# bigpon/QPNet

Hardware: AMD Instinct MI355X
Metric: train steps/sec (batch-1 chunk-steps of RF+20000 samples, aggregate over GPUs) (higher is better)
Workload: dtype f32; 1 GPU; config[1]: paper-size SI-QPNet (C=64,S=256,4F+4A) training step, forward+CE+backward+Adam on one chunk of 20900 samples (RF 946 + batch_length 19954), batch 1 per GPU; global_batch=1, parallelism=dp1 (utterance-sharded chunks, one flat-gradient all-reduce per step), backend=none, world_size=1, aux_1x1=frame rate (hoisted: K = 128 + one 4-deep step)

## Files before the change

qpnet_amd/csrc/train_common.h:

```cpp
#pragma once
#include "qpn_common.h"

typedef float f32x4 __attribute__((ext_vector_type(4)));

#define TR_MAXL QPN_MAX_LAYERS

__host__ __device__ static inline int tr_lda(int K) { return ((K + 29) / 32) * 32 + 2; }
__host__ __device__ static inline int tr_ldt(int N) { return ((N + 15) / 32) * 32 + 16; }

struct TrLayer {
    int adaptive, dilation;
    int s_in, s_out;
    int tap_off;
    int w1_f4, wr_f4;
    int w1t_f4, wrt_f4;
    int bias1, biasr;
};

struct TrainParams {
    int C, S, Q, A, Ap, L, U;
    int B, T, F, Td, BL, N1, N0, maxd;
    int Kt, Ktp;
    int LC;
    const float* flat;
// ... 21 lines not shown
    int qtotal;
    int qP[TR_MAXL + 1];
    int qT[TR_MAXL];
    int ws_f4, p1_f4, p2_f4;
    int wst_f4, p1t_f4, p2t_f4;
    int bias_s, bias_p1, bias_p2;
    int64_t causal_w, causal_b, up_w, up_b;
    TrLayer layers[TR_MAXL];
};

struct TrainSlabs {
    int g_w1[TR_MAXL], g_b1[TR_MAXL], g_wr[TR_MAXL], g_br[TR_MAXL], g_ws[TR_MAXL], g_bs;
    int g_p1, g_bp1, g_p2, g_bp2;
    int g_early0, g_early1;
    int g_cw, g_cb;
};

struct TrainBwd {
    const float* dlogits; float* gflat;
    float* DXA[2]; float* DXB[2];
    float* DZ;
    float* DS0; float* DY0;
    float* DGS;
    float* DHUP;
    float* DPA;
    float* GW;
    float* EB;
    float* slab;
    const int* gdst; const int* gdst_list;
    const int* gzero; int n_gzero;
    int nch, gstage;
    int64_t n_params;
    const struct TrainSlabs* sl;
    float gscale;
    int append_scale;
    const int* status;
    hipStream_t side; hipEvent_t ev_fork, ev_join, ev_mid;
    hipEvent_t ev_early; int* early_recorded;
};


struct AuxGeom { int auxS[TR_MAXL], auxT[TR_MAXL], bias1[TR_MAXL], s_out[TR_MAXL]; };
struct AuxArgs {
    const float* flat; const float* h; float* PA; float* bp; const float* DPA; const float* EB; const float* GW; float* gflat;
    float gscale; int C, A, L, B, F, U, N1, nfr, ffirst; int64_t up_w, up_b;
    AuxGeom g;
};
static inline AuxArgs tr_aux_args(const TrainParams& p, const TrainBwd* bw, const AuxGeom& ag) {
    AuxArgs a; a.flat = p.flat; a.h = p.h; a.PA = p.PA; a.bp = p.bp; a.DPA = bw ? bw->DPA : nullptr; a.EB = bw ? bw->EB : nullptr; a.GW = bw ? bw->GW : nullptr;
    a.gflat = bw ? bw->gflat : nullptr; a.gscale = bw ? bw->gscale : 1.f;
    a.C = p.C; a.A = p.A; a.L = p.L; a.B = p.B; a.F = p.F; a.U = p.U; a.N1 = p.N1; a.nfr = p.nfr; a.ffirst = p.ffirst; a.up_w = p.up_w; a.up_b = p.up_b; a.g = ag;
    return a;
}
struct TrainKnobs {
    bool serial;
    bool stack_q_fwd, stack_q_bwd;
    int stack_wgs, stack_wgs_bwd;
    bool persist_fwd, persist_bwd;
    bool wgrad_generic;
    int wgrad_chunks, wgrad_chunks_side;
    bool post_fuse;
    bool up_side, reduce_early, wr_side;
    bool post_pair, zero_in_post, post_wide;
    bool xcd_swizzle;
    bool ce_separate;
    bool event_fence;
    bool aux_hoist;
    bool test_stack_gives_up;
};
void qpn_train_knobs_parse(TrainKnobs& k);

#define TR_QHEAD_STRIDE 1056
#define TR_QHDR_WORDS 17920
struct StackQ {
    unsigned* flags;
    unsigned* head;
    unsigned* stats;
    unsigned* abort;
    const int4* tab;
    unsigned epoch;
    unsigned epoch_pub;
    unsigned spin_limit;
    int total, nq;
};

__host__ __device__ __forceinline__ int tr_pa_off(const TrainParams& p, int l, int b, int n0) {
    const int q = p.F * p.U - p.N1 + n0;
    return ((l * p.B + b) * (p.nfr + 1) + (q / p.U - p.ffirst)) * 2 * p.C;
}

__device__ __forceinline__ void tr_queue_entry_fwd(const TrainParams& p, int pos, int4& a, int4& b) {
    const bool valid = pos < p.qtotal;
    const int ps = valid ? pos : 0;
    int l = 0;
    for (int k = 1; k < p.L; ++k) l += ps >= p.qP[k] ? 1 : 0;
    const int r = ps - p.qP[l], T = p.qT[l];
    const int bi = r / T, t = r - bi * T;
    const TrLayer ly = p.layers[l];
    const int n0 = ly.s_out + 16 * t;
    int first = 0, n = 0;
    if (valid && l > 0) {
        const int reach = ly.s_out - ly.s_in, s_prev = p.layers[l - 1].s_out;
        int lo = n0 - reach; if (lo < s_prev) lo = s_prev;
        int hi = n0 + 15; if (hi > p.N1 - 1) hi = p.N1 - 1;
        const int t_lo = (lo - s_prev) >> 4, t_hi = (hi - s_prev) >> 4;
        first = p.qP[l - 1] + bi * p.qT[l - 1] + t_lo; n = t_hi - t_lo + 1;
    }
    a = make_int4(n0, l | (bi << 8) | (l == p.L - 1 ? 1 << 24 : 0) | (valid ? 1 << 25 : 0), first, n);
    b = make_int4((l * p.B + bi) * p.N1, ly.tap_off + bi * p.N1, p.hoist ? tr_pa_off(p, l, bi, n0) : bi * p.N1, 0);
}

__device__ __forceinline__ void tr_queue_entry_bwd(const TrainParams& p, int pos, int4& a, int4& b) {
    const bool valid = pos < p.qtotal;
    const int ps = valid ? pos : 0;
    int k = 0, base = 0;
    for (int j = 0; j + 1 < p.L; ++j) { const int n = p.B * p.qT[p.L - 1 - j]; if (ps >= base + n) { base += n; k = j + 1; } else break; }
    const int l = p.L - 1 - k;
    const int r = ps - base, T = p.qT[l];
    const int bi = r / T, t = r - bi * T;
// ... 233 lines not shown
```

qpnet_amd/csrc/train_fwd.hip:

```cpp
#include "train_common.h"
#include "train_post.h"

__device__ __forceinline__ float sigmoidf_(float z) { return __builtin_amdgcn_rcpf(1.0f + __expf(-z)); }
__device__ __forceinline__ float tanhf_(float z) { return 2.0f * __builtin_amdgcn_rcpf(1.0f + __expf(-2.0f * z)) - 1.0f; }

#define AUXP_FPB 8
__device__ __forceinline__ void aux_proj_block(const TrainParams& p, const AuxGeom& ag, int fxb, int l, int b, float* sm) {
    const int fx0 = fxb * AUXP_FPB, tid = threadIdx.x, n = tid & 127, fh = tid >> 7, C = p.C, A = p.A, CA = C * A;
    float* Va = sm; float* hs = sm + 2 * CA;
    {
        const float* s0 = p.flat + ag.auxS[l]; const float* s1 = p.flat + ag.auxT[l];
        for (int base = 0; base < 2 * CA; base += 256 * 16) {
            float v[16];
#pragma unroll
            for (int k = 0; k < 16; ++k) { const int i = base + 256 * k + tid, ic = i < 2 * CA ? i : 0; v[k] = ic < CA ? s0[ic] : s1[ic - CA]; }
#pragma unroll
            for (int k = 0; k < 16; ++k) { const int i = base + 256 * k + tid; if (i < 2 * CA) Va[i] = v[k]; }
        }
    }
    for (int i = tid; i < A * AUXP_FPB; i += 256) {
        const int a = i / AUXP_FPB, f = i - a * AUXP_FPB, fx = fx0 + f;
        hs[i] = fx < p.nfr ? p.h[((size_t)b * A + a) * p.F + p.ffirst + fx] : 0.f;
    }
    __syncthreads();
    float acc[4] = {0.f, 0.f, 0.f, 0.f}, vs = 0.f;
    for (int a = 0; a < A; ++a) {
        const float v = Va[n * A + a];
        const float4 h4 = *(const float4*)(hs + a * AUXP_FPB + 4 * fh);
        acc[0] += v * h4.x; acc[1] += v * h4.y; acc[2] += v * h4.z; acc[3] += v * h4.w;
        vs += v;
    }
    float* out = p.PA + ((size_t)(l * p.B + b) * (p.nfr + 1) + fx0 + 4 * fh) * 2 * C + n;
#pragma unroll
    for (int f = 0; f < 4; ++f) if (fx0 + 4 * fh + f <= p.nfr) out[(size_t)f * 2 * C] = acc[f];
    if (fxb == 0 && b == 0 && fh == 0) p.bp[ag.bias1[l] + n] += p.flat[p.up_b] * vs;
}

__global__ __launch_bounds__(256) void k_train_prep(TrainParams p, AuxGeom ag, int nprep) {
    const int b = blockIdx.y;
    if ((int)blockIdx.x >= nprep) {
        extern __shared__ float sm[];
        const int idx = blockIdx.x - nprep, nfxb = (p.nfr + 1 + AUXP_FPB - 1) / AUXP_FPB;
        aux_proj_block(p, ag, idx % nfxb, idx / nfxb, b, sm);
        return;
    }
    const int C = p.C, Q = p.Q, N1 = p.N1, Ap = p.Ap;
    const int C4 = C / 4, A4 = Ap / 4;
    const int nX = N1 * C4, nH = p.hoist ? 0 : N1 * A4;
    const int total = nX + nH + N1 * p.L;
    if (p.hoist && b == 0)
        for (int n = blockIdx.x * 256 + threadIdx.x; n < N1 + 16; n += nprep * 256) {
            const int q = p.F * p.U - N1 + n, j = q - (q / p.U) * p.U;
            p.WJ[n] = make_float2(p.flat[p.up_w + j], __int_as_float(j));
        }
    if (p.qctl && blockIdx.x == 0 && b == 0 && threadIdx.x < 32) p.qctl[threadIdx.x < 16 ? threadIdx.x : 1024 + (threadIdx.x - 16) * TR_QHEAD_STRIDE] = 0u;
    if (p.qtab && b == 0)
        for (int pos = blockIdx.x * 256 + threadIdx.x; pos <= p.qtotal; pos += nprep * 256) {
            int4 ea, eb; tr_queue_entry_fwd(p, pos, ea, eb);
            p.qtab[2 * pos] = ea; p.qtab[2 * pos + 1] = eb;
            if (p.qtab_b) { tr_queue_entry_bwd(p, pos, ea, eb); p.qtab_b[2 * pos] = ea; p.qtab_b[2 * pos + 1] = eb; }
        }
    for (int it = blockIdx.x * 256 + threadIdx.x; it < total; it += nprep * 256) {
        if (it < nX) {
            const int n = it / C4, c = (it - n * C4) * 4;
            const int64_t xo = (int64_t)p.T - p.N0 + n;
            int64_t s0 = p.x[(size_t)b * p.T + xo] % Q, s1 = p.x[(size_t)b * p.T + xo + 1] % Q;
            if (s0 < 0) s0 += Q;
            if (s1 < 0) s1 += Q;
            const float4 r0 = *(const float4*)(p.ct + (size_t)s0 * C + c);
            const float4 r1 = *(const float4*)(p.ct + ((size_t)Q + s1) * C + c);
            const float4 bb = *(const float4*)(p.flat + p.causal_b + c);
            float4 v;
            v.x = (r0.x + r1.x) + bb.x; v.y = (r0.y + r1.y) + bb.y; v.z = (r0.z + r1.z) + bb.z; v.w = (r0.w + r1.w) + bb.w;
            *(float4*)(p.X + ((size_t)b * N1 + n) * C + c) = v;
            if (c == 0) { p.XC[(size_t)b * (N1 + 1) + n] = (int)s0; if (n == N1 - 1) p.XC[(size_t)b * (N1 + 1) + N1] = (int)s1; }
        } else if (it < nX + nH) {
            const int i2 = it - nX, n = i2 / A4, a0 = (i2 - n * A4) * 4;
            float v[4];
            int64_t f = 0; int j = 0;
            if (p.U > 0) { const int64_t q = (int64_t)p.F * p.U - N1 + n; f = q / p.U; j = (int)(q - f * p.U); }
            else f = (int64_t)p.F - N1 + n;
            const float wj = p.U > 0 ? p.flat[p.up_w + j] : 1.0f, ub = p.U > 0 ? p.flat[p.up_b] : 0.0f;
#pragma unroll
            for (int e = 0; e < 4; ++e) {
                const int a = a0 + e;
                float t = 0.0f;
                if (a < p.A) { t = p.h[((size_t)b * p.A + a) * p.F + f]; if (p.U > 0) t = t * wj + ub; }
                v[e] = t;
            }
            *(float4*)(p.HUP + ((size_t)b * N1 + n) * Ap + a0) = make_float4(v[0], v[1], v[2], v[3]);
        } else {
            const int i3 = it - nX - nH, l = i3 / N1, n = i3 - l * N1;
            const TrLayer ly = p.layers[l];
            int tap;
            if (ly.adaptive) {
                const float dv = p.d[(size_t)b * p.Td + (p.Td - N1 + n)];
                const float dil = -dv * (float)ly.dilation;
                const float s = __fadd_rn(dil, (float)(n - N1));
                tap = N1 + (int)rintf(s);
                if (n >= ly.s_out && (tap < ly.s_in || tap > n)) { atomicOr(p.status, 1); }
            } else tap = n - ly.dilation;
            tap = tap < 0 ? 0 : (tap >= N1 ? N1 - 1 : tap);
            p.TAP[ly.tap_off + (size_t)b * N1 + n] = tap;
        }
    }
}

template <int MT>
__device__ __forceinline__ void layer_fwd_tile(const TrainParams& p, const int l, const int last, const int b, const int n0, float* sm) {
    constexpr int TM = 16 * MT;
    const TrLayer ly = p.layers[l];
    const int C = p.C, Ktp = p.Ktp, Ap = p.Ap;
    const int lda = tr_lda(Ktp), ldg = tr_lda(C);
    float* As = sm; float* Gs = sm + TM * lda;
    const int tid = threadIdx.x, lane = tid & 63, wave = tid >> 6;
    const float* Xin = p.X + ((size_t)(l * p.B + b) * p.N1) * C;
    const float* hup = p.HUP + (size_t)b * p.N1 * Ap;
    const int* taps = p.TAP + ly.tap_off + (size_t)b * p.N1;
    const float* bias1 = p.bp + ly.bias1;
    const float* br = p.bp + ly.biasr;
    const int cpre = 16 * (wave < C / 16 ? wave : 0) + (lane & 15);
    const float bs_pre = bias1[cpre], bt_pre = bias1[C + cpre], bb_pre = br[cpre];
    float4 wrq[4][1];
    if (!last) { const int ntp[1] = {wave < C / 16 ? wave : 0}; wave_b_preload<1, 4>(wrq, p.wp + ly.wr_f4, C / 16, ntp, C, lane); }
    {
        const int K4 = Ktp / 4;
        const int tpr = K4 < 64 ? K4 : 64;
        const int rpp = 256 / tpr;
        const int tr = tid / tpr, tc = tid - tr * tpr;
        constexpr int NR = TM / 4;
        if (tr < rpp) {
            int tp[NR];
#pragma unroll
            for (int k = 0; k < NR; ++k) {
                const int n = n0 + tr + k * rpp;
                tp[k] = taps[n < p.N1 ? n : p.N1 - 1];
            }
            for (int c4 = tc; c4 < K4; c4 += tpr) {
                const int k0 = c4 * 4;
                const int kind = k0 < C ? 0 : k0 < 2 * C ? 1 : k0 < 2 * C + Ap ? 2 : 3;
                const bool from_x = kind <= 1;
                const int col = kind == 0 ? k0 : kind == 1 ? k0 - C : kind == 2 ? k0 - 2 * C : 0;
                const unsigned long long ax = (unsigned long long)Xin, ah = (unsigned long long)hup;
                const float* base = (const float*)(from_x ? ax : ah) + col;
                const int stride = from_x ? C : Ap;
                float4 v[NR];
#pragma unroll
                for (int k = 0; k < NR; ++k) {
                    const int r = tr + k * rpp, n = n0 + r;
                    const bool ok = r < TM && n < p.N1 && kind != 3;
                    const int row = ok ? (kind == 1 ? tp[k] : n) : 0;
                    v[k] = *(const float4*)(base + (size_t)row * stride);
                }
                __builtin_amdgcn_sched_barrier(0);
#pragma unroll
                for (int k = 0; k < NR; ++k) {
                    const int r = tr + k * rpp;
                    if (r < TM) {
// ... 437 lines not shown
    post_fwd_w_tile<MT, false>(p, sm, mS, mY, bq);
}

__global__ __launch_bounds__(256) void k_ce(const float* __restrict__ logits, const int64_t* __restrict__ tgt, int64_t tgt_stride,
                                            int BL, int Q, int64_t rows, float* __restrict__ dlogits, double* __restrict__ loss, int rpw, int* __restrict__ status) {
    __shared__ double part[4];
    const int lane = threadIdx.x & 63, wave = threadIdx.x >> 6;
    const float inv = 1.0f / (float)rows;
    double lsum = 0.0;
    for (int it = 0; it < rpw; ++it) {
        const int64_t row = ((int64_t)blockIdx.x * rpw + it) * 4 + wave;
        if (row >= rows) break;
        const float* lg = logits + (size_t)row * Q;
        const int64_t b = row / BL, t = row - b * BL;
        int64_t tg = tgt[(size_t)b * tgt_stride + (tgt_stride - BL) + t];
        if (tg < 0 || tg >= Q) { if (lane == 0) atomicOr(status, 2); tg = tg < 0 ? 0 : Q - 1; }
        float m = -INFINITY;
        const bool vec = (Q & 255) == 0;
        if (vec) for (int q = lane * 4; q < Q; q += 256) { const float4 v = *(const float4*)(lg + q); m = fmaxf(fmaxf(m, fmaxf(v.x, v.y)), fmaxf(v.z, v.w)); }
        else for (int q = lane; q < Q; q += 64) m = fmaxf(m, lg[q]);
        m = tr_wave_max(m);
        float se = 0.f;
        if (vec) for (int q = lane * 4; q < Q; q += 256) { const float4 v = *(const float4*)(lg + q); se += (__expf(v.x - m) + __expf(v.y - m)) + (__expf(v.z - m) + __expf(v.w - m)); }
        else for (int q = lane; q < Q; q += 64) se += expf(lg[q] - m);
        se = tr_wave_sum(se);
        const float lse = logf(se) + m;
        if (dlogits) {
            if (vec) for (int q = lane * 4; q < Q; q += 256) {
                const float4 v = *(const float4*)(lg + q);
                float4 g = make_float4(__expf(v.x - lse), __expf(v.y - lse), __expf(v.z - lse), __expf(v.w - lse));
                const int dq = (int)tg - q;
                if (dq == 0) g.x -= 1.0f; else if (dq == 1) g.y -= 1.0f; else if (dq == 2) g.z -= 1.0f; else if (dq == 3) g.w -= 1.0f;
                *(float4*)(dlogits + (size_t)row * Q + q) = make_float4(g.x * inv, g.y * inv, g.z * inv, g.w * inv);
            } else for (int q = lane; q < Q; q += 64) {
                const float pr = expf(lg[q] - lse);
                dlogits[(size_t)row * Q + q] = (pr - (q == tg ? 1.0f : 0.0f)) * inv;
            }
        }
        lsum += (double)(lse - lg[tg]);
    }
    if (lane == 0) part[wave] = lsum;
    __syncthreads();
    if (threadIdx.x == 0) atomicAdd(loss + (blockIdx.x & 63), (part[0] + part[1] + part[2] + part[3]) / (double)rows);
}

void qpn_launch_prep(const TrainParams& p, const AuxGeom& ag, hipStream_t stream) {
    const long items = (long)p.N1 * (p.C / 4 + (p.hoist ? 0 : p.Ap / 4) + p.L);
    const int blocks = (int)((items + 255) / 256 < 4096 ? (items + 255) / 256 : 4096);
    const int naux = p.hoist ? (p.nfr + 1 + AUXP_FPB - 1) / AUXP_FPB * p.L : 0;
    const size_t lds = p.hoist ? (size_t)(2 * p.C * p.A + p.A * AUXP_FPB + 8) * sizeof(float) : 0;
    hipLaunchKernelGGL(k_train_prep, dim3(blocks + naux, p.B), dim3(256), lds, stream, p, ag, blocks);
}

bool qpn_stack_fwd_fits(const TrainParams& p);
int qpn_launch_stack_fwd(const TrainParams& p, const StackQ& q, const TrainKnobs& k, hipStream_t stream);

void qpn_launch_post_fb(const TrainParams& p, const TrainBwd& bw, hipStream_t stream);

int qpn_launch_fwd(const TrainParams& p, const TrainKnobs& k, const AuxGeom& ag, const StackQ* sq, hipStream_t stream, const TrainBwd* fuse_post_bwd) {
    const int C = p.C, S = p.S;
    qpn_launch_prep(p, ag, stream);
    qpn_prof_mark(PG_PREP, stream);
    const size_t lds_layer = (size_t)16 * (tr_lda(p.Ktp) + tr_lda(C)) * sizeof(float);
    const size_t lds_post = (size_t)16 * (tr_lda(S) + (tr_lda(S) > 2 * tr_lda(C) ? tr_lda(S) : 2 * tr_lda(C))) * sizeof(float);
    if (lds_layer > 160 * 1024 || lds_post > 160 * 1024) {
        qpn_set_error("training kernels: tiles do not fit the 160 KiB LDS for n_resch=%d n_skipch=%d (n_resch <= 128 supported)", C, S);
        return QPN_EINVAL;
    }
    {
        const int flags0 = k.xcd_swizzle ? 2 : 0;
        const bool persist = C == 64 && (p.Ktp == 176 || p.hoist) && p.N1 < (1 << 24) && k.persist_fwd;
        if (p.hoist && !persist) { qpn_set_error("internal: the frame-rate aux term needs the register-resident layer kernels"); return QPN_EINVAL; }
        const bool stack_q = persist && k.stack_q_fwd && sq && sq->flags && p.qctl && qpn_stack_fwd_fits(p);
        if (stack_q) {
            const int rcq = qpn_launch_stack_fwd(p, *sq, k, stream);
            if (rcq) return rcq;
        }
        for (int l = 0; l < p.L && !stack_q; ++l) {
            const int rows = p.N1 - p.layers[l].s_out;
            const int tiles = (rows + 15) / 16;
            if (persist) {
                int G = qpn_num_cus() * 2; if (G > tiles) G = tiles;
                if (G > 1024) G = 1024;
                const size_t ldsp = (size_t)(32 * tr_lda(p.Ktp) + 4 * 16 * tr_lda(64)) * sizeof(float);
                const bool last = l == p.L - 1;
                if (p.hoist) {
                    if (last) hipLaunchKernelGGL((k_layer_fwd_p<8, true>), dim3(G, p.B), dim3(256), ldsp, stream, p, l, flags0, tiles, p.scratch_rows);
                    else hipLaunchKernelGGL((k_layer_fwd_p<8, false>), dim3(G, p.B), dim3(256), ldsp, stream, p, l, flags0, tiles, p.scratch_rows);
                } else {
                    if (last) hipLaunchKernelGGL((k_layer_fwd_p<11, true>), dim3(G, p.B), dim3(256), ldsp, stream, p, l, flags0, tiles, p.scratch_rows);
                    else hipLaunchKernelGGL((k_layer_fwd_p<11, false>), dim3(G, p.B), dim3(256), ldsp, stream, p, l, flags0, tiles, p.scratch_rows);
                }
            } else {
                if (lds_layer > 48 * 1024) (void)hipFuncSetAttribute((const void*)k_layer_fwd<1>, hipFuncAttributeMaxDynamicSharedMemorySize, (int)lds_layer);
                hipLaunchKernelGGL((k_layer_fwd<1>), dim3(tiles, p.B), dim3(256), lds_layer, stream, p, l, (l == p.L - 1 ? 1 : 0) | flags0);
            }
        }
    }
    qpn_prof_mark(PG_LAYER_FWD, stream);
    const bool post_wide = S == 256 && p.Q == 256 && C == 64 && k.post_wide;
    if (post_wide && fuse_post_bwd) qpn_launch_post_fb(p, *fuse_post_bwd, stream);
    else if (post_wide) {
        constexpr int MTW = 5;
        const size_t ldsw = (size_t)16 * MTW * (tr_lda(256) + 2 * tr_lda(64)) * sizeof(float);
        QPN_HIP(hipFuncSetAttribute((const void*)k_post_fwd_w<MTW>, hipFuncAttributeMaxDynamicSharedMemorySize, (int)ldsw));
        hipLaunchKernelGGL((k_post_fwd_w<MTW>), dim3((p.BL + 16 * MTW - 1) / (16 * MTW), p.B), dim3(512), ldsw, stream, p);
    } else {
        if (lds_post > 48 * 1024) (void)hipFuncSetAttribute((const void*)k_post_fwd<1>, hipFuncAttributeMaxDynamicSharedMemorySize, (int)lds_post);
        hipLaunchKernelGGL((k_post_fwd<1>), dim3((p.BL + 15) / 16, p.B), dim3(512), lds_post, stream, p);
    }
    qpn_prof_mark(PG_POST_FWD, stream);
    QPN_HIP(hipGetLastError());
    return QPN_OK;
}
// ... 11 lines not shown
```

qpnet_amd/csrc/train_host.hip:

```cpp
#include "train_common.h"
#include "qpn_handle.h"
#include <algorithm>
#include <string.h>

int qpn_launch_fwd(const TrainParams& p, const TrainKnobs& k, const AuxGeom& ag, const StackQ* sq, hipStream_t stream, const TrainBwd* fuse_post_bwd);
void qpn_stack_fill(TrainParams& p);
int qpn_launch_ce(const float* logits, const int64_t* tgt, int64_t tgt_stride, int B, int BL, int Q, float* dlogits, double* loss, int* status, bool loss_cleared, hipStream_t stream);
int qpn_launch_bwd(const TrainParams& p, const TrainBwd& bw, const TrainKnobs& k, const AuxGeom& ag, const StackQ* sq, hipStream_t stream, bool post_done);
int qpn_launch_fwd_gemm(const TrainParams& p, const TrainGemm& w, hipStream_t stream);
int qpn_launch_bwd_gemm(const TrainParams& p, const TrainBwd& bw, const TrainGemm& w, hipStream_t stream);
int qpn_launch_adam(float* w, const float* g, float* m, float* v, int64_t n, int step, float lr, float b1, float b2, float eps, float wd, const float* den, int* status,
                    int* h_status, double* h_loss, const double* d_loss, float* e, float omd, hipStream_t stream);
int qpn_launch_adam_clip(float* w, const float* g, float* m, float* v, int64_t n, int step, float lr, float b1, float b2, float eps, float wd, const float* den, int* status,
                         int* h_status, double* h_loss, const double* d_loss, float max_norm, double* part, double* d_norm, double* h_norm, float* e, float omd, hipStream_t stream);
int qpn_launch_grad_accum(float* acc, const float* g, int64_t cnt, int first, const int* status, int* h_status, double* h_loss, const double* d_loss, hipStream_t stream);

#define LOSS_SLOT 72

struct TrainState {
    std::vector<int> h_wmap;
    std::vector<int> h_bstart, h_blist;
    std::vector<int> h_gsrc;
    int* d_wmap; float* d_wp; int* d_bstart; int* d_blist; float* d_bp; int n_bias;
    int* d_gdst; int* d_gdst_list; int* d_gzero; int n_gzero;
    bool hoist;
    TrainParams tp;
    TrainBwd bw;
    TrainSlabs slabs;
    TrainKnobs knobs;
    AuxGeom ag;
    float* d_ws; size_t ws_cap;
    int* d_tap; size_t tap_cap;
    int* d_status; double* d_loss;
    hipStream_t last_stream;
    int* h_status_pinned; hipEvent_t ev_status[2]; bool status_pending[2]; int status_newest;
    double* h_loss_pinned; hipEvent_t ev_loss[2]; bool loss_pending[2]; int loss_newest;
    double* d_gnorm; bool gnorm_last;
    bool gnorm_slot[2];
    double gnorm_collected; bool gnorm_collected_valid;
    bool fwd_valid;
    bool loss_clear;
    bool use_gemm;
    int* d_ctmap; float* d_ct;
    std::vector<int> h_gmap; int* d_gmap; float* d_gwp;
    TrainGemm gm;
    int64_t generation;
    hipStream_t side; hipEvent_t ev_fork, ev_join, ev_mid;
    hipEvent_t ev_early; int early_recorded; int64_t early_first;
    int64_t bwd_generation;
    const float* post_bwd_dlogits;
    bool post_bwd_done;
    bool stack_disabled;
    unsigned* d_sq; size_t sq_pos_cap, sq_per_dir;
    StackQ sqf, sqb;
};

static int env_int(const char* name, int dflt) { const char* e = getenv(name); return (e && *e) ? atoi(e) : dflt; }
void qpn_train_knobs_parse(TrainKnobs& k) {
    k.serial = env_int("QPN_TRAIN_SERIAL", 0) != 0;
    k.stack_q_fwd = env_int("QPN_STACK_QUEUE", 1) != 0;
    k.stack_q_bwd = k.stack_q_fwd && env_int("QPN_STACK_QUEUE_BWD", 1) != 0;
    k.stack_wgs = env_int("QPN_STACK_WGS", 0); if (k.stack_wgs < 0 || k.stack_wgs > 4096) k.stack_wgs = 0;
    k.stack_wgs_bwd = env_int("QPN_STACK_WGS_BWD", 0); if (k.stack_wgs_bwd < 0 || k.stack_wgs_bwd > 4096) k.stack_wgs_bwd = 0;
    k.persist_fwd = env_int("QPN_LAYER_PERSIST", 1) != 0;
    k.persist_bwd = env_int("QPN_LAYER_BWD_PERSIST", 1) != 0;
    k.wgrad_generic = getenv("QPN_WGRAD_GENERIC") != nullptr;
    k.wgrad_chunks = env_int("QPN_WGRAD_CHUNKS", 0); if (k.wgrad_chunks < 1 || k.wgrad_chunks > 512) k.wgrad_chunks = 0;
    k.wgrad_chunks_side = env_int("QPN_WGRAD_CHUNKS_SIDE", 0); if (k.wgrad_chunks_side < 1 || k.wgrad_chunks_side > 512) k.wgrad_chunks_side = 0;
    k.up_side = env_int("QPN_UP_SIDE", 1) != 0;
    k.reduce_early = env_int("QPN_REDUCE_EARLY", 1) != 0;
    k.wr_side = env_int("QPN_WR_SIDE", 1) != 0;
    k.post_fuse = env_int("QPN_POST_FUSE", 1) != 0;
    k.post_pair = env_int("QPN_POST_WGRAD_PAIR", 1) != 0;
    k.zero_in_post = env_int("QPN_ZERO_IN_POST", 1) != 0;
    k.post_wide = env_int("QPN_POST_WIDE", 1) != 0;
    k.xcd_swizzle = getenv("QPN_NO_XCD_SWIZZLE") == nullptr;
    k.ce_separate = getenv("QPN_CE_SEPARATE") != nullptr;
    k.event_fence = env_int("QPN_EVENT_FENCE", 0) == 1;
    k.aux_hoist = env_int("QPN_AUX_HOIST", 1) != 0;
    k.test_stack_gives_up = false;
#ifdef QPN_TESTING
    k.test_stack_gives_up = env_int("QPN_TEST_STACK_GIVES_UP", 0) == 1;
#endif
}

int qpn_num_cus() {
    static int cached[64] = {0};
    int dev = 0;
    if (hipGetDevice(&dev) != hipSuccess || dev < 0 || dev >= 64) return 256;
    if (!cached[dev]) { int n = 0; if (hipDeviceGetAttribute(&n, hipDeviceAttributeMultiprocessorCount, dev) != hipSuccess || n < 1) n = 256; cached[dev] = n; }
    return cached[dev];
}

struct Prof { bool on = false; bool overlapped = false; std::vector<hipEvent_t> ev; std::vector<int> grp; std::vector<hipStream_t> st; size_t used = 0; };
static thread_local Prof g_prof;
bool qpn_prof_active() { return g_prof.on; }
bool qpn_prof_serial() { return g_prof.on && !g_prof.overlapped; }
void qpn_prof_mark(int group, hipStream_t stream) {
    Prof& P = g_prof;
    if (!P.on) return;
    if (P.used == P.ev.size()) { hipEvent_t e; if (hipEventCreate(&e) != hipSuccess) return; P.ev.push_back(e); P.grp.push_back(0); P.st.push_back(nullptr); }
    P.grp[P.used] = group; P.st[P.used] = stream;
    (void)hipEventRecord(P.ev[P.used++], stream);
}
extern "C" int qpn_train_profile_begin(qpn_handle* h, void* stream) {
    (void)h; g_prof.on = true; g_prof.overlapped = false; g_prof.used = 0;
    qpn_prof_mark(-1, (hipStream_t)stream);
    return QPN_OK;
}
extern "C" int qpn_train_profile_begin_overlapped(qpn_handle* h, void* stream) {
    (void)h; g_prof.on = true; g_prof.overlapped = true; g_prof.used = 0;
    qpn_prof_mark(-1, (hipStream_t)stream);
    return QPN_OK;
}
extern "C" int qpn_train_profile_mark(qpn_handle* h, int group, void* stream) {
    (void)h; qpn_prof_mark(group, (hipStream_t)stream); return QPN_OK;
}
extern "C" int qpn_train_profile_end(qpn_handle* h, float* h_ms, int n, void* stream) {
    Prof& P = g_prof;
    QPN_HIP(hipStreamSynchronize((hipStream_t)stream));
    if (h && h->train && h->train->side) QPN_HIP(hipStreamSynchronize(h->train->side));
    for (int i = 0; i < n; ++i) h_ms[i] = 0.f;
    for (size_t i = 1; i < P.used; ++i) {
        if (P.grp[i] < 0 || P.grp[i] >= n) continue;
        size_t j = i;
        while (j > 0 && P.st[j - 1] != P.st[i]) --j;
        if (j == 0) continue;
        float ms = 0.f;
        QPN_HIP(hipEventElapsedTime(&ms, P.ev[j - 1], P.ev[i]));
        h_ms[P.grp[i]] += ms;
    }
    P.on = false;
// ... 322 lines not shown
    const size_t nScr = (size_t)B * 1024 * 2 * 128;
    size_t need = nScr + nX + 2 * nG + nH + 2 * (nS + 96 * (size_t)S + 64) + 2 * (size_t)(L + 1) * nDX + (size_t)L * nDZ + 2 * nS + nDGS + nH + nSlab + nXC + (t->use_gemm ? nG : 0) + 2 * nPA + nWJ + nGW + (size_t)L * TR_EB_SLOTS * 2 * C + 8192;
    if (need > t->ws_cap) {
        if (t->d_ws) (void)hipFree(t->d_ws);
        t->d_ws = nullptr; t->ws_cap = 0;
        hipError_t e = hipMalloc(&t->d_ws, need * sizeof(float));
        if (e != hipSuccess) { qpn_set_error("hipMalloc(%zu MiB) for the training workspace failed", need * 4 >> 20); return QPN_ENOMEM; }
        t->ws_cap = need;
    }
    const size_t ntap = (size_t)std::max(nA, 1) * B * N1;
    if (ntap > t->tap_cap) {
        if (t->d_tap) (void)hipFree(t->d_tap);
        t->d_tap = nullptr; t->tap_cap = 0;
        QPN_HIP(hipMalloc(&t->d_tap, ntap * sizeof(int)));
        t->tap_cap = ntap;
    }
    float* w = t->d_ws;
    auto carve = [&](size_t n) { float* r = w; w += (n + 63) & ~(size_t)63; return r; };
    p.X = carve(nX); p.SG = carve(nG); p.TH = carve(nG); p.HUP = carve(nH); p.S0 = carve(nS + 96 * (size_t)S); p.Y0 = carve(nS + 96 * (size_t)S);
    bw.DXA[0] = carve((size_t)(L + 1) * nDX); bw.DXB[0] = carve((size_t)(L + 1) * nDX); bw.DXA[1] = bw.DXB[1] = nullptr;
    bw.DZ = carve((size_t)L * nDZ); bw.DS0 = carve(nS); bw.DY0 = carve(nS); bw.DGS = carve(nDGS); bw.DHUP = carve(nH); bw.slab = carve(nSlab);
    p.XC = (int*)carve(nXC);
    p.scratch_rows = carve(nScr);
    if (t->use_gemm) t->gm.G = carve(nG);
    p.PA = nullptr; p.WJ = nullptr; bw.DPA = nullptr; bw.GW = nullptr;
    bw.EB = nullptr;
    if (t->hoist) { p.PA = carve(nPA); bw.DPA = carve(nPA + (size_t)L * TR_EB_SLOTS * 2 * C); bw.EB = bw.DPA + nPA; p.WJ = (float2*)carve(nWJ); bw.GW = carve(nGW); }
    p.TAP = t->d_tap; p.status = t->d_status;
    t->last_stream = stream;
    {
        qpn_stack_fill(p);
        if ((size_t)p.qtotal > t->sq_pos_cap) {
            if (t->d_sq) (void)hipFree(t->d_sq);
            t->d_sq = nullptr; t->sq_pos_cap = 0;
            const size_t cap = (size_t)p.qtotal + (size_t)p.qtotal / 2 + 64;
            const size_t per_dir = (cap / 32 + 2) * 1056;
            const size_t nsq = TR_QHDR_WORDS + 2 * per_dir + 2 * (cap + 1) * 8;
            QPN_HIP(hipMalloc(&t->d_sq, nsq * sizeof(unsigned)));
            QPN_HIP(hipMemsetAsync(t->d_sq, 0, nsq * sizeof(unsigned), stream));
            t->sq_pos_cap = cap; t->sq_per_dir = per_dir;
        }
        hipStreamCaptureStatus cap_st = hipStreamCaptureStatusNone;
        (void)hipStreamIsCapturing(stream, &cap_st);
        const bool no_queue = t->stack_disabled || cap_st != hipStreamCaptureStatusNone;
        p.qctl = no_queue ? nullptr : t->d_sq;
        p.qtab = no_queue ? nullptr : (int4*)(t->d_sq + TR_QHDR_WORDS + 2 * t->sq_per_dir);
        p.qtab_b = no_queue ? nullptr : p.qtab + 2 * (t->sq_pos_cap + 1);
        const unsigned epoch = (unsigned)((t->generation + 1) % 0xFFFFFFFFll) + 1u;
        StackQ& f = t->sqf; StackQ& bq = t->sqb;
        f.flags = t->d_sq + TR_QHDR_WORDS; f.head = t->d_sq + 1024; f.abort = t->d_sq + 1; f.stats = t->d_sq + 4; f.epoch = epoch; f.total = p.qtotal; f.tab = p.qtab;
        bq.flags = f.flags + t->sq_per_dir; bq.head = f.head + 8 * TR_QHEAD_STRIDE; bq.abort = f.abort; bq.stats = t->d_sq + 8; bq.epoch = epoch; bq.total = p.qtotal; bq.tab = p.qtab_b;
    }
    p.flat = d_flat; p.wp = (const float4*)t->d_wp; p.bp = t->d_bp; p.x = d_x; p.h = d_h; p.d = d_dfac; p.logits = d_logits;
    {
        const int* wmap = t->use_gemm ? t->d_gmap : t->d_wmap;
        float* wout = t->use_gemm ? t->d_gwp : t->d_wp;
        const int64_t nw = (int64_t)(t->use_gemm ? t->h_gmap.size() : t->h_wmap.size()), nct = (int64_t)2 * g.Q * g.C;
        const int64_t tot = nw + nct + t->n_bias + 16 + 64;
        hipLaunchKernelGGL(k_refresh, dim3((unsigned)((tot + 255) / 256)), dim3(256), 0, stream, d_flat, wmap, wout, nw, t->d_ctmap, t->d_ct, nct,
                           t->d_bstart, t->d_blist, t->d_bp, t->n_bias, t->d_status, t->d_loss);
        p.ct = t->d_ct;
    }
    qpn_prof_mark(PG_PREP, stream);
    t->fwd_valid = false; t->loss_clear = true;
    ++t->generation;
    const bool fuse_ce = d_targets && !t->use_gemm && g.Q <= g.S && g.Q % 256 == 0 && !t->knobs.ce_separate;
    p.ce_tgt = fuse_ce ? d_targets : nullptr; p.ce_stride = tgt_stride; p.ce_dlogits = d_dlogits; p.ce_loss = t->d_loss;
    if (fuse_ce && !want_logits) p.logits = nullptr;
    const bool fuse_post = fuse_bwd && fuse_ce && d_dlogits && t->knobs.post_fuse && t->knobs.post_wide && t->knobs.zero_in_post && g.S == 256 && g.Q == 256 && g.C == 64 && (p.LC == 256 || p.LC == 512);
    t->post_bwd_done = false;
    rc = t->use_gemm ? qpn_launch_fwd_gemm(p, t->gm, stream) : qpn_launch_fwd(p, t->knobs, t->ag, &t->sqf, stream, fuse_post ? &t->bw : nullptr);
    if (!rc) { t->post_bwd_done = fuse_post; t->post_bwd_dlogits = d_dlogits; }
    p.ce_tgt = nullptr; p.logits = d_logits;
    if (rc) return rc;
    t->fwd_valid = true;
    if (fuse_ce) { t->loss_clear = false; qpn_prof_mark(PG_CE, stream); }
    else if (d_targets) {
        rc = qpn_launch_ce(d_logits, d_targets, tgt_stride, B, BL, g.Q, d_dlogits, t->d_loss, t->d_status, t->loss_clear, stream); if (rc) return rc;
        t->loss_clear = false;
    }
    return QPN_OK;
}

extern "C" int qpn_train_forward(qpn_handle* h, const float* d_flat, int B, int64_t T, int64_t F, int64_t Td, int BL, int maxd,
                                 const int64_t* d_x, const float* d_h, const float* d_dfac, float* d_logits, void* stream_) {
    return train_forward_impl(h, d_flat, B, T, F, Td, BL, maxd, d_x, d_h, d_dfac, d_logits, nullptr, 0, nullptr, 1, stream_);
}

extern "C" int qpn_train_forward_loss(qpn_handle* h, const float* d_flat, int B, int64_t T, int64_t F, int64_t Td, int BL, int maxd,
                                      const int64_t* d_x, const float* d_h, const float* d_dfac, const int64_t* d_targets, int64_t tgt_stride,
                                      float* d_logits, int want_logits, float* d_dlogits, void* stream_) {
    if (!d_targets) { qpn_set_error("bad train_forward_loss arguments: no targets"); return QPN_EINVAL; }
    return train_forward_impl(h, d_flat, B, T, F, Td, BL, maxd, d_x, d_h, d_dfac, d_logits, d_targets, tgt_stride, d_dlogits, want_logits & 1, stream_, (want_logits & QPN_FWD_BACKWARD_FOLLOWS) != 0);
}

extern "C" int qpn_train_loss(qpn_handle* h, double* h_loss, void* stream_) {
    int rc = need_dev(h); if (rc) return rc;
    if (!h->train || !h_loss) { qpn_set_error("qpn_train_loss needs a preceding qpn_train_forward_loss / qpn_ce_loss"); return QPN_ESTATE; }
    hipStream_t stream = (hipStream_t)stream_;
    double parts[64];
    QPN_HIP(hipMemcpyAsync(parts, h->train->d_loss, sizeof(parts), hipMemcpyDeviceToHost, stream));
    QPN_HIP(hipStreamSynchronize(stream));
    double sum = 0.0;
    for (int i = 0; i < 64; ++i) sum += parts[i];
    *h_loss = sum;
    return QPN_OK;
}

extern "C" int qpn_train_loss_enqueue(qpn_handle* h, void* stream_) {
    int rc = need_dev(h); if (rc) return rc;
    if (!h->train) { qpn_set_error("qpn_train_loss_enqueue needs a preceding qpn_train_forward_loss / qpn_ce_loss"); return QPN_ESTATE; }
    TrainState* t = h->train;
    const int slot = t->loss_newest ^ 1;
    if (t->loss_pending[slot]) QPN_HIP(hipEventSynchronize(t->ev_loss[slot]));
    QPN_HIP(hipMemcpyAsync(t->h_loss_pinned + LOSS_SLOT * slot, t->d_loss, (t->gnorm_last ? 65 : 64) * sizeof(double), hipMemcpyDeviceToHost, (hipStream_t)stream_));
    t->gnorm_slot[slot] = t->gnorm_last;
    QPN_HIP(hipEventRecord(t->ev_loss[slot], (hipStream_t)stream_));
    t->loss_pending[slot] = true; t->loss_newest = slot;
    return QPN_OK;
}
extern "C" int qpn_train_loss_collect(qpn_handle* h, int newest, double* h_loss, int* h_valid) {
    int rc = need_dev(h); if (rc) return rc;
    if (!h_loss || !h_valid) { qpn_set_error("bad loss_collect arguments"); return QPN_EINVAL; }
    *h_valid = 0; *h_loss = 0.0;
// ... 358 lines not shown
```

Measured before the change: 1474 steps/s.

## Fuse weight refresh, bias refresh and training prep into one step-prep kernel

Merges the separate k_refresh launch (weight repack, causal-table build, bias sums, loss clear) with k_train_prep into a single k_step_prep kernel whose block ranges cover each job. The causal embedding is now computed directly from the causal weights staged in LDS per channel slice, so the intermediate ct table is no longer built. The aux bias term is folded into the bias refresh instead of being accumulated with +=. This removes one kernel launch and its serialization barrier per step, at the cost of a more complex heterogeneous kernel with a larger LDS requirement.

Result: faster. 1493 steps/s, median of 6 (+1.2%).

```diff
diff --git a/qpnet_amd/csrc/train_common.h b/qpnet_amd/csrc/train_common.h
--- a/qpnet_amd/csrc/train_common.h
+++ b/qpnet_amd/csrc/train_common.h
@@ -97,6 +97,7 @@
     a.C = p.C; a.A = p.A; a.L = p.L; a.B = p.B; a.F = p.F; a.U = p.U; a.N1 = p.N1; a.nfr = p.nfr; a.ffirst = p.ffirst; a.up_w = p.up_w; a.up_b = p.up_b; a.g = ag;
     return a;
 }
+struct RefreshArgs { const int* wmap; float* wout; int64_t nw; const int* bstart; const int* blist; int nb; double* loss; };
 struct TrainKnobs {
     bool serial;
     bool stack_q_fwd, stack_q_bwd;
@@ -110,6 +111,7 @@
     bool xcd_swizzle;
     bool ce_separate;
     bool event_fence;
+    bool prep_fuse;
     bool aux_hoist;
     bool test_stack_gives_up;
 };
diff --git a/qpnet_amd/csrc/train_fwd.hip b/qpnet_amd/csrc/train_fwd.hip
--- a/qpnet_amd/csrc/train_fwd.hip
+++ b/qpnet_amd/csrc/train_fwd.hip
@@ -5,6 +5,7 @@
 __device__ __forceinline__ float tanhf_(float z) { return 2.0f * __builtin_amdgcn_rcpf(1.0f + __expf(-2.0f * z)) - 1.0f; }
 
 #define AUXP_FPB 8
+template <bool BIAS>
 __device__ __forceinline__ void aux_proj_block(const TrainParams& p, const AuxGeom& ag, int fxb, int l, int b, float* sm) {
     const int fx0 = fxb * AUXP_FPB, tid = threadIdx.x, n = tid & 127, fh = tid >> 7, C = p.C, A = p.A, CA = C * A;
     float* Va = sm; float* hs = sm + 2 * CA;
@@ -33,35 +34,29 @@
     float* out = p.PA + ((size_t)(l * p.B + b) * (p.nfr + 1) + fx0 + 4 * fh) * 2 * C + n;
 #pragma unroll
     for (int f = 0; f < 4; ++f) if (fx0 + 4 * fh + f <= p.nfr) out[(size_t)f * 2 * C] = acc[f];
-    if (fxb == 0 && b == 0 && fh == 0) p.bp[ag.bias1[l] + n] += p.flat[p.up_b] * vs;
-}
-
-__global__ __launch_bounds__(256) void k_train_prep(TrainParams p, AuxGeom ag, int nprep) {
-    const int b = blockIdx.y;
-    if ((int)blockIdx.x >= nprep) {
-        extern __shared__ float sm[];
-        const int idx = blockIdx.x - nprep, nfxb = (p.nfr + 1 + AUXP_FPB - 1) / AUXP_FPB;
-        aux_proj_block(p, ag, idx % nfxb, idx / nfxb, b, sm);
-        return;
-    }
+    if (BIAS && fxb == 0 && b == 0 && fh == 0) p.bp[ag.bias1[l] + n] += p.flat[p.up_b] * vs;
+}
+
+template <bool X0>
+__device__ __forceinline__ void prep_items(const TrainParams& p, const int bx, const int nprep, const int b) {
     const int C = p.C, Q = p.Q, N1 = p.N1, Ap = p.Ap;
     const int C4 = C / 4, A4 = Ap / 4;
     const int nX = N1 * C4, nH = p.hoist ? 0 : N1 * A4;
     const int total = nX + nH + N1 * p.L;
     if (p.hoist && b == 0)
-        for (int n = blockIdx.x * 256 + threadIdx.x; n < N1 + 16; n += nprep * 256) {
+        for (int n = bx * 256 + threadIdx.x; n < N1 + 16; n += nprep * 256) {
             const int q = p.F * p.U - N1 + n, j = q - (q / p.U) * p.U;
             p.WJ[n] = make_float2(p.flat[p.up_w + j], __int_as_float(j));
         }
-    if (p.qctl && blockIdx.x == 0 && b == 0 && threadIdx.x < 32) p.qctl[threadIdx.x < 16 ? threadIdx.x : 1024 + (threadIdx.x - 16) * TR_QHEAD_STRIDE] = 0u;
+    if (p.qctl && bx == 0 && b == 0 && threadIdx.x < 32) p.qctl[threadIdx.x < 16 ? threadIdx.x : 1024 + (threadIdx.x - 16) * TR_QHEAD_STRIDE] = 0u;
     if (p.qtab && b == 0)
-        for (int pos = blockIdx.x * 256 + threadIdx.x; pos <= p.qtotal; pos += nprep * 256) {
+        for (int pos = bx * 256 + threadIdx.x; pos <= p.qtotal; pos += nprep * 256) {
             int4 ea, eb; tr_queue_entry_fwd(p, pos, ea, eb);
             p.qtab[2 * pos] = ea; p.qtab[2 * pos + 1] = eb;
             if (p.qtab_b) { tr_queue_entry_bwd(p, pos, ea, eb); p.qtab_b[2 * pos] = ea; p.qtab_b[2 * pos + 1] = eb; }
         }
-    for (int it = blockIdx.x * 256 + threadIdx.x; it < total; it += nprep * 256) {
-        if (it < nX) {
+    for (int it = (X0 ? 0 : nX) + bx * 256 + threadIdx.x; it < total; it += nprep * 256) {
+        if (X0 && it < nX) {
             const int n = it / C4, c = (it - n * C4) * 4;
             const int64_t xo = (int64_t)p.T - p.N0 + n;
             int64_t s0 = p.x[(size_t)b * p.T + xo] % Q, s1 = p.x[(size_t)b * p.T + xo + 1] % Q;
@@ -104,6 +99,115 @@
             p.TAP[ly.tap_off + (size_t)b * N1 + n] = tap;
         }
     }
+}
+__global__ __launch_bounds__(256) void k_train_prep(TrainParams p, AuxGeom ag, int nprep) {
+    const int b = blockIdx.y;
+    if ((int)blockIdx.x >= nprep) {
+        extern __shared__ float sm[];
+        const int idx = blockIdx.x - nprep, nfxb = (p.nfr + 1 + AUXP_FPB - 1) / AUXP_FPB;
+        aux_proj_block<true>(p, ag, idx % nfxb, idx / nfxb, b, sm);
+        return;
+    }
+    prep_items<true>(p, blockIdx.x, nprep, b);
+}
+
+#ifndef X0_CS
+#define X0_CS 16
+#define X0_ST 17
+#endif
+#define X0_RPG 512
+struct StepPrepPlan { int nx0, rpg, naux, nbias, nwt, nprep; };
+
+__device__ __forceinline__ void x0_block(const TrainParams& p, const int blk, const int rpg, float* sm) {
+    const int C = p.C, Q = p.Q, N1 = p.N1, tid = threadIdx.x;
+    const int nsl = C / X0_CS, grp = blk / nsl, c0 = (blk - grp * nsl) * X0_CS;
+    const int R = p.B * N1, r0 = grp * rpg, nr = R - r0 < rpg ? R - r0 : rpg;
+    float* tab = sm; int* cls = (int*)(sm + 2 * Q * X0_ST);
+    const float4* src = (const float4*)(p.flat + p.causal_w + (size_t)c0 * Q * 2);
+    const int n4 = X0_CS * Q / 2;
+    const float bb = p.flat[p.causal_b + c0 + (tid & (X0_CS - 1))];
+    for (int base = 0; base < n4; base += 256 * 8) {
+        float4 v[8];
+#pragma unroll
+        for (int k = 0; k < 8; ++k) { const int e4 = base + 256 * k + tid; v[k] = src[e4 < n4 ? e4 : 0]; }
+        if (base == 0)
+            for (int j = tid; j < nr; j += 256) {
+                const int r = r0 + j, b = r / N1, n = r - b * N1;
+                const int64_t xo = (int64_t)p.T - p.N0 + n;
+                int64_t s0 = p.x[(size_t)b * p.T + xo] % Q, s1 = p.x[(size_t)b * p.T + xo + 1] % Q;
+                if (s0 < 0) s0 += Q;
+                if (s1 < 0) s1 += Q;
+                cls[j] = (int)s0; cls[rpg + j] = (int)s1;
+            }
+#pragma unroll
+        for (int k = 0; k < 8; ++k) {
+            const int e4 = base + 256 * k + tid;
+            if (e4 < n4) {
+                const int e = 4 * e4, cl = e / (2 * Q), q = (e - cl * 2 * Q) >> 1;
+                float* d = tab + q * X0_ST + cl;
+                d[0] = v[k].x; d[Q * X0_ST] = v[k].y; d[X0_ST] = v[k].z; d[(Q + 1) * X0_ST] = v[k].w;
+            }
+        }
+    }
+    __syncthreads();
+    const int c = tid & (X0_CS - 1);
+    for (int j = tid / X0_CS; j < nr; j += 256 / X0_CS) {
+        const int s0 = cls[j], s1 = cls[rpg + j], r = r0 + j;
+        p.X[(size_t)r * C + c0 + c] = (tab[s0 * X0_ST + c] + tab[(Q + s1) * X0_ST + c]) + bb;
+        if (c0 == 0 && c == 0) {
+            const int b = r / N1, n = r - b * N1;
+            p.XC[(size_t)b * (N1 + 1) + n] = s0; if (n == N1 - 1) p.XC[(size_t)b * (N1 + 1) + N1] = s1;
+        }
+    }
+}
+
+__global__ __launch_bounds__(256) void k_step_prep(TrainParams p, AuxGeom ag, RefreshArgs rf, StepPrepPlan pl) {
+    extern __shared__ float sm[];
+    int blk = blockIdx.x;
+    const int tid = threadIdx.x;
+    if (blk < pl.nx0) { x0_block(p, blk, pl.rpg, sm); return; }
+    blk -= pl.nx0;
+    if (blk < pl.naux) {
+        const int nfxb = (p.nfr + 1 + AUXP_FPB - 1) / AUXP_FPB, per_b = nfxb * p.L, b = blk / per_b, idx = blk - b * per_b;
+        aux_proj_block<false>(p, ag, idx % nfxb, idx / nfxb, b, sm);
+        return;
+    }
+    blk -= pl.naux;
+    if (blk < pl.nbias) {
+        const int i = blk * 256 + tid, C = p.C, A = p.A;
+        if (i >= rf.nb) { if (i < rf.nb + 64) rf.loss[i - rf.nb] = 0.0; return; }
+        int lg = -1, ng = 0;
+        if (p.hoist) for (int l = 0; l < p.L; ++l) { const int n = i - ag.bias1[l]; if (n >= 0 && n < 2 * C) { lg = l; ng = n; } }
+        float va[64];
+        if (lg >= 0) {
+            const float* s = p.flat + (ng < C ? ag.auxS[lg] + ng * A : ag.auxT[lg] + (ng - C) * A);
+#pragma unroll
+            for (int a = 0; a < 64; ++a) va[a] = s[a < A ? a : 0];
+        }
+        float acc = 0.f;
+        for (int j = rf.bstart[i]; j < rf.bstart[i + 1]; ++j) acc += p.flat[rf.blist[j]];
+        if (lg >= 0) {
+            float vs = 0.f;
+#pragma unroll
+            for (int a = 0; a < 64; ++a) if (a < A) vs += va[a];
+            acc += p.flat[p.up_b] * vs;
+        }
+        p.bp[i] = acc;
+        return;
+    }
+    blk -= pl.nbias;
+    if (blk < pl.nwt) {
+        const int64_t i4 = (int64_t)blk * 256 + tid, i = i4 * 4;
+        if (i + 4 <= rf.nw) {
+            const int4 m = ((const int4*)rf.wmap)[i4];
+            const float t0 = p.flat[m.x >= 0 ? m.x : 0], t1 = p.flat[m.y >= 0 ? m.y : 0], t2 = p.flat[m.z >= 0 ? m.z : 0], t3 = p.flat[m.w >= 0 ? m.w : 0];
+            ((float4*)rf.wout)[i4] = make_float4(m.x >= 0 ? t0 : 0.f, m.y >= 0 ? t1 : 0.f, m.z >= 0 ? t2 : 0.f, m.w >= 0 ? t3 : 0.f);
+        } else for (int64_t k = i; k < rf.nw; ++k) { const int m = rf.wmap[k]; rf.wout[k] = m >= 0 ? p.flat[m] : 0.0f; }
+        return;
+    }
+    blk -= pl.nwt;
+    const int b = blk / pl.nprep;
+    prep_items<false>(p, blk - b * pl.nprep, pl.nprep, b);
 }
 
 template <int MT>
@@ -647,14 +751,41 @@
     hipLaunchKernelGGL(k_train_prep, dim3(blocks + naux, p.B), dim3(256), lds, stream, p, ag, blocks);
 }
 
+static size_t step_prep_lds_x0(const TrainParams& p, int rpg) { return ((size_t)2 * p.Q * X0_ST + 2 * (size_t)rpg) * sizeof(float); }
+static int step_prep_rpg(const TrainParams& p) {
+    const int64_t R = (int64_t)p.B * p.N1;
+    const int64_t rpg = (R + 127) / 128;
+    return (int)(rpg < 16 ? 16 : rpg > X0_RPG ? X0_RPG : rpg);
+}
+bool qpn_step_prep_fits(const TrainParams& p) {
+    if (p.C % X0_CS || p.Q % 2 || p.causal_w % 4 || ((uintptr_t)p.flat & 15) || (p.hoist && p.A > 64)) return false;
+    return step_prep_lds_x0(p, X0_RPG) <= 40 * 1024;
+}
+void qpn_launch_step_prep(const TrainParams& p, const AuxGeom& ag, const RefreshArgs& rf, hipStream_t stream) {
+    StepPrepPlan pl;
+    pl.rpg = step_prep_rpg(p);
+    pl.nx0 = (int)(((int64_t)p.B * p.N1 + pl.rpg - 1) / pl.rpg) * (p.C / X0_CS);
+    pl.naux = p.hoist ? (p.nfr + 1 + AUXP_FPB - 1) / AUXP_FPB * p.L * p.B : 0;
+    pl.nbias = (rf.nb + 64 + 255) / 256;
+    pl.nwt = (int)((rf.nw + 1023) / 1024);
+    const long items = (long)p.N1 * ((p.hoist ? 0 : p.Ap / 4) + p.L);
+    pl.nprep = (int)((items + 255) / 256 < 4096 ? (items + 255) / 256 : 4096);
+    if (pl.nprep < 1) pl.nprep = 1;
+    size_t lds = step_prep_lds_x0(p, pl.rpg);
+    const size_t lds_aux = p.hoist ? (size_t)(2 * p.C * p.A + p.A * AUXP_FPB + 8) * sizeof(float) : 0;
+    if (lds_aux > lds) lds = lds_aux;
+    hipLaunchKernelGGL(k_step_prep, dim3((unsigned)(pl.nx0 + pl.naux + pl.nbias + pl.nwt + pl.nprep * p.B)), dim3(256), lds, stream, p, ag, rf, pl);
+}
+
 bool qpn_stack_fwd_fits(const TrainParams& p);
 int qpn_launch_stack_fwd(const TrainParams& p, const StackQ& q, const TrainKnobs& k, hipStream_t stream);
 
 void qpn_launch_post_fb(const TrainParams& p, const TrainBwd& bw, hipStream_t stream);
 
-int qpn_launch_fwd(const TrainParams& p, const TrainKnobs& k, const AuxGeom& ag, const StackQ* sq, hipStream_t stream, const TrainBwd* fuse_post_bwd) {
+int qpn_launch_fwd(const TrainParams& p, const TrainKnobs& k, const AuxGeom& ag, const StackQ* sq, hipStream_t stream, const TrainBwd* fuse_post_bwd, const RefreshArgs* rf) {
     const int C = p.C, S = p.S;
-    qpn_launch_prep(p, ag, stream);
+    if (rf) qpn_launch_step_prep(p, ag, *rf, stream);
+    else qpn_launch_prep(p, ag, stream);
     qpn_prof_mark(PG_PREP, stream);
     const size_t lds_layer = (size_t)16 * (tr_lda(p.Ktp) + tr_lda(C)) * sizeof(float);
     const size_t lds_post = (size_t)16 * (tr_lda(S) + (tr_lda(S) > 2 * tr_lda(C) ? tr_lda(S) : 2 * tr_lda(C))) * sizeof(float);
diff --git a/qpnet_amd/csrc/train_host.hip b/qpnet_amd/csrc/train_host.hip
--- a/qpnet_amd/csrc/train_host.hip
+++ b/qpnet_amd/csrc/train_host.hip
@@ -3,7 +3,8 @@
 #include <algorithm>
 #include <string.h>
 
-int qpn_launch_fwd(const TrainParams& p, const TrainKnobs& k, const AuxGeom& ag, const StackQ* sq, hipStream_t stream, const TrainBwd* fuse_post_bwd);
+int qpn_launch_fwd(const TrainParams& p, const TrainKnobs& k, const AuxGeom& ag, const StackQ* sq, hipStream_t stream, const TrainBwd* fuse_post_bwd, const RefreshArgs* rf);
+bool qpn_step_prep_fits(const TrainParams& p);
 void qpn_stack_fill(TrainParams& p);
 int qpn_launch_ce(const float* logits, const int64_t* tgt, int64_t tgt_stride, int B, int BL, int Q, float* dlogits, double* loss, int* status, bool loss_cleared, hipStream_t stream);
 int qpn_launch_bwd(const TrainParams& p, const TrainBwd& bw, const TrainKnobs& k, const AuxGeom& ag, const StackQ* sq, hipStream_t stream, bool post_done);
@@ -78,6 +79,7 @@
     k.ce_separate = getenv("QPN_CE_SEPARATE") != nullptr;
     k.event_fence = env_int("QPN_EVENT_FENCE", 0) == 1;
     k.aux_hoist = env_int("QPN_AUX_HOIST", 1) != 0;
+    k.prep_fuse = env_int("QPN_PREP_FUSE", 1) != 0;
     k.test_stack_gives_up = false;
 #ifdef QPN_TESTING
     k.test_stack_gives_up = env_int("QPN_TEST_STACK_GIVES_UP", 0) == 1;
@@ -506,13 +508,18 @@
         bq.flags = f.flags + t->sq_per_dir; bq.head = f.head + 8 * TR_QHEAD_STRIDE; bq.abort = f.abort; bq.stats = t->d_sq + 8; bq.epoch = epoch; bq.total = p.qtotal; bq.tab = p.qtab_b;
     }
     p.flat = d_flat; p.wp = (const float4*)t->d_wp; p.bp = t->d_bp; p.x = d_x; p.h = d_h; p.d = d_dfac; p.logits = d_logits;
+    RefreshArgs rf;
+    bool fuse_prep;
     {
         const int* wmap = t->use_gemm ? t->d_gmap : t->d_wmap;
         float* wout = t->use_gemm ? t->d_gwp : t->d_wp;
         const int64_t nw = (int64_t)(t->use_gemm ? t->h_gmap.size() : t->h_wmap.size()), nct = (int64_t)2 * g.Q * g.C;
         const int64_t tot = nw + nct + t->n_bias + 16 + 64;
-        hipLaunchKernelGGL(k_refresh, dim3((unsigned)((tot + 255) / 256)), dim3(256), 0, stream, d_flat, wmap, wout, nw, t->d_ctmap, t->d_ct, nct,
-                           t->d_bstart, t->d_blist, t->d_bp, t->n_bias, t->d_status, t->d_loss);
+        rf.wmap = wmap; rf.wout = wout; rf.nw = nw; rf.bstart = t->d_bstart; rf.blist = t->d_blist; rf.nb = t->n_bias; rf.loss = t->d_loss;
+        fuse_prep = t->knobs.prep_fuse && !t->use_gemm && qpn_step_prep_fits(p);
+        if (!fuse_prep)
+            hipLaunchKernelGGL(k_refresh, dim3((unsigned)((tot + 255) / 256)), dim3(256), 0, stream, d_flat, wmap, wout, nw, t->d_ctmap, t->d_ct, nct,
+                               t->d_bstart, t->d_blist, t->d_bp, t->n_bias, t->d_status, t->d_loss);
         p.ct = t->d_ct;
     }
     qpn_prof_mark(PG_PREP, stream);
@@ -523,7 +530,7 @@
     if (fuse_ce && !want_logits) p.logits = nullptr;
     const bool fuse_post = fuse_bwd && fuse_ce && d_dlogits && t->knobs.post_fuse && t->knobs.post_wide && t->knobs.zero_in_post && g.S == 256 && g.Q == 256 && g.C == 64 && (p.LC == 256 || p.LC == 512);
     t->post_bwd_done = false;
-    rc = t->use_gemm ? qpn_launch_fwd_gemm(p, t->gm, stream) : qpn_launch_fwd(p, t->knobs, t->ag, &t->sqf, stream, fuse_post ? &t->bw : nullptr);
+    rc = t->use_gemm ? qpn_launch_fwd_gemm(p, t->gm, stream) : qpn_launch_fwd(p, t->knobs, t->ag, &t->sqf, stream, fuse_post ? &t->bw : nullptr, fuse_prep ? &rf : nullptr);
     if (!rc) { t->post_bwd_done = fuse_post; t->post_bwd_dlogits = d_dlogits; }
     p.ce_tgt = nullptr; p.logits = d_logits;
     if (rc) return rc;
```
